# daac-tools/daachorse

Hardware: AMD Instinct MI355X
Metric: haystack GB/s scanned (find_overlapping_iter(..).count(), 100k-pattern bytewise automaton) (higher is better)
Workload: dtype u8/u32 integer

## Files before the change

### daachorse_amd/csrc/device_tables.hpp

```cpp
#pragma once

#include <hip/hip_runtime.h>

#include <cstdint>

#include "../../include/daachorse_amd.h"

namespace daac {

struct TierDev {
    const void *rows;
    const uint32_t *bcmap;
    const uint32_t *bfail;
    const uint2 *ssum;
    const uint8_t *cls;
    const uint4 *grec;
    const uint32_t *sopos;
    const uint32_t *outputs;
    const uint32_t *ohash;
    uint32_t C, NA, NB, N;
    uint32_t off_bcmap, off_bfail, off_ssum, off_cls, lds_bytes;
    uint32_t row32, root_flag;
};

struct DArrayDev {
    const uint2 *hot;
    const uint32_t *fail;
    const uint32_t *fail_plain;
    const uint4 *rec;
    const uint4 *root_chain;
    const uint4 *root;
    const uint2 *osum;
    const uint32_t *outputs;
    const uint32_t *ohash;
    uint32_t n, root_flag, leftmost;
};

struct CharDev {
    const uint4 *states;
    const uint32_t *fail_plain;
    const uint32_t *table;
    const uint2 *osum;
    const uint32_t *outputs;
    const uint32_t *ohash;
    uint32_t table_len, n, root_flag, leftmost;
    uint32_t map_in_lds;
    uint32_t map_lo;
    const uint2 *root_row;
    uint32_t alphabet;
    uint32_t row_in_lds;
    const uint4 *wstates;
    uint32_t obits, fbits;
};

struct ScanArgs {
    const uint8_t *hay;
    uint64_t begin;
    uint64_t len;
    uint64_t seg_bytes;
    uint64_t nseg;
    uint32_t halo;
    unsigned long long *result;
    unsigned long long *seg_counts;
    daac_match *out;
    uint64_t total_len;
    unsigned long long *flags;
};

struct ScanArgs;
struct ChainArgs;

struct ChainArgs {
    const unsigned long long *x_spec;
    const unsigned long long *x_prev;
    unsigned long long *x_out;
    unsigned int *flags;
    uint4 *tally_spec;
    uint4 *tally_delta;
    uint64_t cap;
};

struct GramDev {
    const uint32_t *cls32;
    const uint16_t *cid;
    const uint2 *combo;
    const uint32_t *bbits;
    const uint8_t *brank;
    const uint32_t *bsuper;
    const uint4 *drec;
    const uint2 *dhit;
    const uint4 *dhit4;
    const uint32_t *cfirst;
    uint32_t off_cid, off_combo, off_bbits, off_brank, off_bsuper, off_scratch, lds_bytes;
    uint32_t K, C, CC, CCC;
    uint32_t level_start, unused_byte, has_short;
    uint32_t rank_in_lds;
    uint32_t n_deep;
};

struct GramArgs {
    const uint8_t *hay_al;
    uint32_t lead;
    uint64_t vlen;
    uint64_t region_bytes;
    uint64_t nregions;
    unsigned long long *result;
    uint2 *wq;
    uint32_t wq_slab;
    uint32_t ppl;
    uint32_t dense;
    const uint32_t *sel;
    uint32_t sel_want;
};

hipError_t launch_gram_scan(const GramDev &dev, const GramArgs &a, uint32_t blocks, uint32_t threads, hipStream_t stream);

constexpr uint32_t kGram2OffH = 512;
struct Gram2Dev {
    const uint8_t *cls;
    const uint32_t *m;
    const void *sdir;
    const uint16_t *rfull;
    const uint16_t *cid4;
    const uint32_t *hsum;
    const uint4 *drec;
    const uint2 *dhit;
    const uint4 *dhit4;
    const uint32_t *cfirst;
    uint32_t m_bytes, s_bytes, cid_bytes, h_bytes;
    uint32_t off_m_count, off_s_count, off_ring_count, lds_count;
    uint32_t rfull_bytes, off_ring_rfull, lds_rfull, rfull_ok;
    uint32_t off_m_exact, off_s_exact, off_cid, off_ring_exact, lds_exact;
    uint32_t K, C, s16, unused_byte, n_deep, exact_ok;
    uint32_t xlane_dpp;
};
uint32_t gram2_lds_bytes(const Gram2Dev &dev, bool exact);

struct Gram2WDev {
    const uint8_t *cls;
    const unsigned long long *m;
    const uint32_t *sdir;
    const uint16_t *cid4;
    const uint32_t *hsum;
    const uint4 *drec;
    const uint4 *dhit;
    uint32_t m_bytes, s_bytes, cid_bytes, h_bytes;
    uint32_t off_m_count, off_s_count, off_ring_count, lds_count;
    uint32_t off_m_exact, off_s_exact, off_cid, off_ring_exact, lds_exact;
    uint32_t C, unused_byte, n_deep, exact_ok;
};
hipError_t launch_gram2w_scan(const Gram2WDev &dev, const GramArgs &a, bool exact, uint32_t blocks, hipStream_t stream);

constexpr uint32_t kGram2OffM = 512;
struct Gram2EmitDev {
    const uint8_t *cls;
    const uint32_t *me;
    const void *sdir;
    const uint32_t *v1, *v2;
    const uint32_t *v3;
    const uint4 *erec;
    const uint2 *ehit;
    const uint4 *ehit4;
    const uint32_t *dupo, *dupv;
    uint32_t level_start;
    const uint32_t *cfirst;
    uint32_t m_bytes, s_bytes, v1_bytes, v2_bytes;
    uint32_t off_s, off_v1, off_v2, off_ring, off_wave, lds_bytes;
    uint32_t K, C, s16, unused_byte;
    const uint32_t *v3c;
    uint32_t v3c_bytes, v3c_dir, v3c_val;
};
hipError_t launch_gram2_scan(const Gram2Dev &dev, const GramArgs &a, bool exact, uint32_t blocks, uint32_t threads, hipStream_t stream);

struct Gram3Lds {
    uint32_t off_s;
    uint32_t off_wave;
    uint32_t wave_stride;
    uint32_t lds_bytes, threads, rfull;
};

constexpr uint32_t kGram4EndsBitDev = 30;
struct Gram4Dev {
    const uint8_t *cls;
    const uint32_t *m;
    const uint16_t *rfull;
    const void *sdir;
    const uint2 *dhit_c;
    const uint4 *dhit_t;
    const uint4 *drec_c;
    const uint4 *drec_t;
    const uint32_t *bloom;
    uint32_t bloom_words;
    uint32_t m_bytes, rfull_bytes, s_bytes;
    uint32_t K, C, s16, arith, lo, unused_byte, n_deep;
};
struct Gram4Lds {
    uint32_t off_wave;
    uint32_t wave_stride;
    uint32_t off_cls;
    uint32_t off_s;
    uint32_t off_m;
    uint32_t s_bytes;
    uint32_t lds_bytes, threads;
    uint32_t arith;
    uint32_t dir;
    uint32_t filter;
    uint32_t off_b;
    uint32_t s_bytes_f;
};
uint32_t gram4_filter_room(uint32_t m_bytes, uint32_t sdir_bytes, bool arith, uint32_t lds_limit);
bool gram4_plan(const Gram4Dev &dev, uint32_t ppl, uint32_t waves, bool rfull, bool want_arith, bool want_filter, uint32_t lds_limit, Gram4Lds &L);
hipError_t launch_gram4_scan(const Gram4Dev &dev, const GramArgs &a, const Gram4Lds &L, uint32_t blocks, hipStream_t stream);

constexpr uint32_t kEmit3Tile = 1024;
constexpr uint32_t kEmit3Chunk = 1024;
constexpr uint32_t kEmit3MaxExtras = 64;
constexpr uint32_t kEmit3Stage = 960;
constexpr uint32_t kEmit3ExpandWave = (kEmit3Stage + 64) * 8 + 2048 + 256 + 1024 + kEmit3MaxExtras * 16 + 16;
constexpr uint32_t kEmit3ExpandWave16 = (kEmit3Stage + 64) * 2 + 1040 + 2048 + 256 + 1024 + kEmit3MaxExtras * 16 + 16;
struct Emit3Args {
    const uint8_t *hay_al;
    uint32_t lead;
    uint32_t vlen;
    uint32_t emit_from;
    uint8_t *ann;
    uint32_t *tile_short;
    uint32_t *tile_deep;
    uint32_t tile0;
    uint4 *recs;
    uint32_t *chunk_fill;
    uint32_t *chunk_next;
    uint32_t chunk_cap;
    uint2 *wq;
    uint32_t wq_slab;
    uint32_t region_bytes;
    uint32_t nregions;
    unsigned int *fail;
};
struct Expand3Args {
    const uint8_t *ann;
    uint32_t ntiles;
    const unsigned long long *tile_off;
    const unsigned long long *bin_off;
    const uint4 *binned;
    void *out;
    unsigned long long pos_base;
    uint32_t off_wave;
    uint32_t has_len1;
    uint32_t v3_in_lds;
    unsigned int *fail;
    uint32_t vlen, emit_from;
};
bool emit3_plan(const Gram2EmitDev &dev, uint32_t waves, uint32_t lds_limit, Gram3Lds &L);
hipError_t launch_emit3_detect(const Gram2EmitDev &dev, const Emit3Args &a, const Gram3Lds &L, uint32_t blocks, hipStream_t stream);
hipError_t launch_emit3_combine(const uint32_t *tile_short, const uint32_t *tile_deep, unsigned long long *total, unsigned long long *deep, uint64_t n,
                                hipStream_t stream);
hipError_t launch_emit3_bin(const uint4 *recs, const uint32_t *chunk_fill, const uint32_t *chunk_next, uint32_t chunk_cap, const unsigned long long *bin_off,
                            uint32_t *cursor, uint4 *binned, uint32_t n1k, unsigned long long rec_limit, uint32_t blocks, hipStream_t stream);
hipError_t launch_emit3_expand(const Gram2EmitDev &dev, const Expand3Args &a, bool f16, uint32_t blocks, hipStream_t stream);
hipError_t launch_emit3_expand_raw(const Gram2EmitDev &dev, const Expand3Args &a, bool f16, uint32_t blocks, hipStream_t stream);
uint32_t emit3_expand_lds_bytes(const Gram2EmitDev &dev, uint32_t waves, bool f16, bool v3_in_lds);

constexpr uint32_t kFind3Tile = 2048;
constexpr uint32_t kFind3Deep = 255;
constexpr uint32_t kLeft3Wave = 2080 + 4096 + 1024 + 256 + 288;
constexpr uint32_t kFind3Wave = 2064 + 4096 + 1024 + 256;
struct Find3Dev {
    const uint32_t *h1, *h2;
    const uint32_t *h3c;
    uint32_t h1_bytes, h2_bytes, h3c_bytes, h3c_dir, h3c_val, C;
};
struct Find3Args {
    const uint8_t *ann;
    uint32_t ntiles;
    uint32_t n1k;
    const unsigned long long *bin_off;
    const uint4 *binned;
    const uint32_t *entry_in;
    uint32_t *exit_out;
    uint32_t force_pos;
    unsigned long long pos_base;
    uint32_t off_wave;
    uint32_t count_only;
    unsigned long long *result;
    unsigned long long *tile_cnt;
    const unsigned long long *tile_off;
    void *out;
    uint32_t f16;
    uint32_t first_start;
    uint32_t last_start;
    uint32_t *last_sel;
    unsigned int *flag;
    const uint32_t *ctl;
    uint32_t chunk_cap;
    unsigned long long rec_limit;
};
__device__ __forceinline__ bool find3_detect_usable(const Find3Args &a) {
    return a.ctl[0] <= a.chunk_cap && a.ctl[1] == 0u && a.bin_off[a.n1k] <= a.rec_limit;
}
uint32_t find3_lds_bytes(const Find3Dev &dev, bool tally);
hipError_t launch_find3_select(const Find3Dev &dev, const Find3Args &a, bool has_len1, bool tally, uint32_t blocks, hipStream_t stream);
hipError_t launch_find3_emit(const Find3Dev &dev, const Find3Args &a, bool has_len1, uint32_t blocks, hipStream_t stream);
hipError_t launch_left3_emit(const Find3Dev &dev, const Find3Args &a, bool has_len1, uint32_t blocks, hipStream_t stream);
hipError_t launch_find3_tail(const Find3Args &a, bool has_len1, uint32_t blocks, hipStream_t stream);
uint32_t left3_lds_bytes(const Find3Dev &dev, bool tally);
hipError_t launch_left3_tail(const Find3Args &a, bool has_len1, uint32_t blocks, hipStream_t stream);
hipError_t launch_left3_select(const Find3Dev &dev, const Find3Args &a, bool has_len1, bool tally, uint32_t blocks, hipStream_t stream);

struct PfxDev {
    const uint32_t *bloom;
    const uint16_t *cnt1;
    const uint16_t *disp;
    const uint4 *slots;
    const uint2 *wrec;
    const uint4 *slots_x;
    const uint4 *wrec_x;
    const uint32_t *hs1;
    const uint4 *slots_e;
    uint32_t G, has_len1, bloom_words, buckets, n_slots, seed;
    uint32_t bloom_bytes, disp_bytes;
    uint32_t off_disp, off_cnt1, off_wave, wave_stride, lds_bytes, threads;
    uint32_t n_keys;
};
bool pfx_plan(PfxDev &d, uint32_t lds_limit);
hipError_t launch_pfx_scan(const PfxDev &dev, const GramArgs &a, bool exact, uint32_t blocks, hipStream_t stream);
hipError_t launch_pfx_probe(const PfxDev &dev, const uint8_t *hay, uint64_t len, unsigned int *out, hipStream_t stream);
struct Emit3Args;
hipError_t launch_pfx_emit_detect(const PfxDev &dev, const Emit3Args &a, uint32_t blocks, hipStream_t stream);

hipError_t launch_overlap_count(const DArrayDev &dev, const ScanArgs &a, bool heads, uint32_t blocks, hipStream_t stream);
hipError_t launch_char_overlap_count(const CharDev &dev, const ScanArgs &a, bool heads, uint32_t blocks, hipStream_t stream);
hipError_t launch_tier_scan(const TierDev &dev, const ScanArgs &a, int mode, bool heads, uint32_t blocks, uint32_t threads,
                            hipStream_t stream);
hipError_t launch_darray_scan(const DArrayDev &dev, const ScanArgs &a, int mode, bool heads, uint32_t blocks, uint32_t threads,
                              hipStream_t stream);
hipError_t launch_restart_scan(const DArrayDev &dev, const ScanArgs &a, int kmode, bool leftmost, unsigned long long *next_begin,
                               uint32_t blocks, uint32_t threads, hipStream_t stream);
hipError_t launch_char_scan(const CharDev &dev, const ScanArgs &a, int mode, bool heads, uint32_t blocks, uint32_t threads,
                            hipStream_t stream);
hipError_t launch_char_restart_scan(const CharDev &dev, const ScanArgs &a, int kmode, bool leftmost, unsigned long long *next_begin,
                                    uint32_t blocks, uint32_t threads, hipStream_t stream);
hipError_t launch_chain(const DArrayDev &dev, const ScanArgs &a, const ChainArgs &c, int pass, int kmode, bool leftmost,
                        unsigned long long *next_begin, uint32_t blocks, hipStream_t stream);
hipError_t launch_char_chain(const CharDev &dev, const ScanArgs &a, const ChainArgs &c, int pass, int kmode, bool leftmost,
                             unsigned long long *next_begin, uint32_t blocks, hipStream_t stream);
hipError_t launch_exclusive_scan(unsigned long long *v, uint64_t n, unsigned long long *total, unsigned long long *scratch, hipStream_t stream);
inline uint64_t exclusive_scan_scratch(uint64_t n) { return n / 2048 + 2; }

}
```

### daachorse_amd/csrc/gram4_kernels.hip

```cpp
#include <hip/hip_runtime.h>

#include <algorithm>
#include <cstdint>
#include <utility>

#include "device_tables.hpp"
#include "gram4_filter.hpp"

namespace daac {

namespace {

typedef uint32_t g4_u32x4_t __attribute__((ext_vector_type(4)));
constexpr uint32_t kList4 = 256;
constexpr uint32_t kProbePercent4 = 3;
typedef __attribute__((address_space(3))) const uint32_t lds4_cu32;
typedef __attribute__((address_space(3))) uint32_t lds4_u32;
typedef __attribute__((address_space(3))) const uint16_t lds4_cu16;
typedef __attribute__((address_space(3))) uint16_t lds4_u16;
typedef __attribute__((address_space(3))) const uint8_t lds4_cu8;
typedef __attribute__((address_space(3))) g4_u32x4_t lds4_u32x4;

__device__ __forceinline__ uint32_t pin4(uint32_t x) {
    asm("" : "+v"(x));
    return x;
}
__device__ __forceinline__ uint32_t mad24(uint32_t a, uint32_t b, uint32_t c) {
    uint32_t d;
    asm("v_mad_u32_u24 %0, %1, %2, %3" : "=v"(d) : "v"(a), "s"(b), "v"(c));
    return d;
}
__device__ __forceinline__ uint32_t wave_shr1_4(uint32_t v, uint32_t lane0) {
    uint32_t d = lane0;
    asm volatile("s_nop 1\nv_mov_b32_dpp %0, %1 wave_shr:1 row_mask:0xf bank_mask:0xf" : "+v"(d) : "v"(v));
    return d;
}
__device__ __forceinline__ uint32_t g4_wave_scan(uint32_t v) {
    v += static_cast<uint32_t>(__builtin_amdgcn_update_dpp(0, static_cast<int>(v), 0x111, 0xf, 0xf, false));
    v += static_cast<uint32_t>(__builtin_amdgcn_update_dpp(0, static_cast<int>(v), 0x112, 0xf, 0xf, false));
    v += static_cast<uint32_t>(__builtin_amdgcn_update_dpp(0, static_cast<int>(v), 0x114, 0xf, 0xf, false));
    v += static_cast<uint32_t>(__builtin_amdgcn_update_dpp(0, static_cast<int>(v), 0x118, 0xf, 0xf, false));
    v += static_cast<uint32_t>(__builtin_amdgcn_update_dpp(0, static_cast<int>(v), 0x142, 0xa, 0xf, false));
    v += static_cast<uint32_t>(__builtin_amdgcn_update_dpp(0, static_cast<int>(v), 0x143, 0xc, 0xf, false));
    return v;
}
template <typename F, int... I>
__device__ __forceinline__ void g4_turns(F &&f, std::integer_sequence<int, I...>) {
    (void)(... && f(std::integral_constant<int, I>{}));
}
__device__ __forceinline__ unsigned long long g4_wave_sum(unsigned long long v) {
#pragma unroll
    for (int off = 32; off > 0; off >>= 1) v += __shfl_down(v, off, 64);
    return v;
}
__device__ __forceinline__ void g4_copy(void *dst, const void *src, uint32_t bytes) {
    const uint4 *s = reinterpret_cast<const uint4 *>(src);
    uint4 *d = reinterpret_cast<uint4 *>(dst);
    for (uint32_t i = threadIdx.x; i < bytes / 16; i += blockDim.x) d[i] = s[i];
}
__device__ __forceinline__ void g4_reduce(unsigned long long cnt, unsigned long long *scratch, unsigned long long *result) {
    const unsigned long long c = g4_wave_sum(cnt);
    __syncthreads();
    const int wave = threadIdx.x >> 6, lane = threadIdx.x & 63;
    if (lane == 0) scratch[wave] = c;
    __syncthreads();
    if (threadIdx.x == 0) {
        unsigned long long r0 = 0;
        for (int w = 0; w < static_cast<int>((blockDim.x + 63) >> 6); ++w) r0 += scratch[w];
        if (r0) atomicAdd(result, r0);
    }
}

}

template <int K, int Q, bool ARITH, int DIR, bool TAIL, bool FILT>
__device__ __forceinline__ void gram4_body(const Gram4Dev &g, const GramArgs &a, const Gram4Lds &L, char *smem) {
    static_assert(!(FILT && TAIL), "the filter runs in front of the plain records");
    static_assert(!(FILT && DIR == 0), "the filter's Bloom array lies where the per-word directory would");
    constexpr int P = 16 * Q;
    constexpr int GS = 8;
    constexpr uint32_t SB = 64u * P;
    constexpr uint32_t SLOT = SB + 32u;
    const uint32_t offM = L.off_m, offS = L.off_s, offC = L.off_cls;
    const uint32_t lo = g.lo, OTH = g.C - 1u, C = g.C;
    auto cls_of = [&](uint32_t byte) -> uint32_t {
        if (ARITH) {
            const uint32_t u = byte - lo;
            return u < OTH ? u : OTH;
        }
        return *reinterpret_cast<lds4_cu8 *>(static_cast<uintptr_t>(offC + byte));
    };
    auto lds_u32 = [&](uint32_t addr) -> uint32_t { return *reinterpret_cast<lds4_cu32 *>(static_cast<uintptr_t>(addr)); };
    auto below = [&](uint32_t k) -> uint32_t { return (1u << k) - 1u; };

    const uint32_t lane = threadIdx.x & 63;
    const uint32_t wave_in_wg = __builtin_amdgcn_readfirstlane(threadIdx.x >> 6);
    const uint32_t C4 = C * 4u, CC4 = C * C * 4u;
    const uint32_t ub4 = g.unused_byte * 0x01010101u;
    const uint8_t *__restrict__ hay = a.hay_al;
    const uint64_t nwaves = static_cast<uint64_t>(gridDim.x) * (blockDim.x >> 6);
    const uint32_t tb = L.off_wave + wave_in_wg * L.wave_stride;
    const uint32_t listb = wave_in_wg * (kList4 * 2u);
    const uint64_t slab_index = (static_cast<uint64_t>(blockIdx.x) * (blockDim.x >> 6) + wave_in_wg) * a.wq_slab;
    uint4 *__restrict__ slab4 = reinterpret_cast<uint4 *>(a.wq) + slab_index;
    uint32_t wq_n = 0, slab_hi = 0;
    uint64_t epoch_base = 0;
    const uint32_t drain_early = wave_in_wg * 64u;

    unsigned long long tot_cnt = 0;
    uint32_t cnt32 = 0;

    auto load_chunk = [&](uint64_t v) -> uint4 {
        if (v >= a.vlen) return uint4{ub4, ub4, ub4, ub4};
        const g4_u32x4_t q = __builtin_nontemporal_load(reinterpret_cast<const g4_u32x4_t *>(hay + v));
        uint4 r{q.x, q.y, q.z, q.w};
        if (v < a.lead || v + 16 > a.vlen) {
            uint32_t w[4] = {r.x, r.y, r.z, r.w};
            for (int b = 0; b < 16; ++b) {
                const uint64_t p = v + b;
                if (p < a.lead || p >= a.vlen) w[b >> 2] = (w[b >> 2] & ~(0xffu << (8 * (b & 3)))) | (g.unused_byte << (8 * (b & 3)));
            }
            r = uint4{w[0], w[1], w[2], w[3]};
        }
        return r;
    };
    auto raw_at = [&](uint64_t p) -> uint32_t { return (p >= a.lead && p < a.vlen) ? hay[p] : g.unused_byte; };
    auto read_ahead = [&](uint64_t v) -> unsigned long long {
        unsigned long long x;
        if (v >= a.lead && v + 8 <= a.vlen) {
            __builtin_memcpy(&x, hay + v, 8);
        } else {
            x = 0;
            for (int b = 7; b >= 0; --b) x = (x << 8) | ((v + b >= a.lead && v + b < a.vlen) ? hay[v + b] : g.unused_byte);
        }
        return x;
    };
    auto tail_count = [&](const uint4 &rr, unsigned long long text) -> uint32_t {
        const uint32_t edges = rr.x & 15u;
        const unsigned long long path = (static_cast<unsigned long long>(rr.w) << 32) | rr.z;
        const unsigned long long diff = path ^ text;
        uint32_t same = diff ? static_cast<uint32_t>(__builtin_ctzll(diff)) >> 3 : 8u;
        same = same < edges ? same : edges;
        return __popc((rr.x >> 4) & ((2u << same) - 1u) & 0x1ffu);
    };
    auto drain = [&]() {
        const uint4 *__restrict__ recs = TAIL ? g.drec_t : g.drec_c;
        uint32_t n_in = wq_n;
        bool raw = !TAIL;
        while (n_in != 0) {
            uint32_t n_out = 0;
            for (uint32_t base = 0; base < n_in; base += 64u) {
                const uint32_t i = base + lane;
                const bool live = i < n_in;
                uint4 e = uint4{0u, 0u, 0u, 0u};
                if (live) e = slab4[i];
                uint32_t state, n_ahead;
                unsigned long long ah;
                if (raw) {
                    const uint32_t k1 = cls_of(e.w & 0xffu);
                    state = e.z + __popc(e.y & below(k1));
                    ah = e.w >> 8;
                    n_ahead = 3;
                } else {
                    state = e.y & 0x07ffffffu;
                    ah = (static_cast<unsigned long long>(e.w & 0xffffffu) << 32) | e.z;
                    n_ahead = e.w >> 24;
                }
                uint4 rr = uint4{0u, 0u, 0u, 0u};
                if (live) rr = recs[state];
                const uint64_t vn = epoch_base + e.x + 2;
                bool cont = false;
                uint32_t next_state = 0;
                if (rr.x >> 31) {
                    if (n_ahead < (rr.x & 15u)) ah = read_ahead(vn);
                    cnt32 += tail_count(rr, ah);
                } else {
                    if (live && n_ahead == 0u) { ah = read_ahead(vn); n_ahead = 8; }
                    const uint32_t k = cls_of(static_cast<uint32_t>(ah) & 0xffu);
                    cnt32 += rr.z;
                    cont = ((rr.x >> k) & 1u) != 0;
                    next_state = rr.y + __popc(rr.x & below(k));
                }
                const unsigned long long m = __ballot(cont);
                if (m != 0) {
                    if (cont) {
                        const uint32_t at = n_out + __builtin_amdgcn_mbcnt_hi(static_cast<uint32_t>(m >> 32), __builtin_amdgcn_mbcnt_lo(static_cast<uint32_t>(m), 0));
                        ah >>= 8;
                        slab4[at] = uint4{e.x + 1u, next_state, static_cast<uint32_t>(ah), static_cast<uint32_t>(ah >> 32) | ((n_ahead - 1u) << 24)};
                    }
                    n_out += static_cast<uint32_t>(__popcll(m));
                }
            }
            n_in = n_out;
            raw = false;
        }
        wq_n = 0;
    };

    uint32_t q_head = 0, q_tail = 0;
    uint32_t posbias = 0;
    uint32_t st_n = 0;
    uint32_t pend_lo = 0;
    uint4 pend = uint4{0u, 0u, 0u, 0u};
    uint32_t pend_pos = 0;
    uint32_t pend_t0 = 0, pend_t1 = 0;
    bool pend_valid = false;
    uint4 p2 = uint4{0u, 0u, 0u, 0u};
    uint32_t p2_pos = 0, p2_state = 0;
    uint32_t p2_t0 = 0, p2_t1 = 0;
    bool p2_live = false, p2_any = false;
    uint32_t sb_n = 0;
    uint32_t sb_pos = 0, sb_lo = 0, sb_t0 = 0;
    uint32_t fp_pos = 0, fp_t0 = 0;
    const uint32_t offB = L.off_b, bloomW = g.bloom_words;
    auto push_walker = [&](bool go, const uint4 &entry) {
        const unsigned long long m = __ballot(go);
        if (m != 0) {
            if (go) {
                const uint32_t at = wq_n + __builtin_amdgcn_mbcnt_hi(static_cast<uint32_t>(m >> 32), __builtin_amdgcn_mbcnt_lo(static_cast<uint32_t>(m), 0));
                slab4[at] = entry;
            }
            wq_n += __popcll(m);
        }
    };
    auto finish_second = [&]() {
        if (!TAIL || !p2_any) return;
        p2_any = false;
        const uint4 r = p2;
        bool again = false;
        uint32_t st_k = 0, pos = p2_pos, t0 = p2_t0, t1n = (p2_t1 & 0xffffffu) | (7u << 24);
        if (p2_live) {
            if (r.x >> 31) {
                if ((r.x & 15u) <= 7u) cnt32 += tail_count(r, (static_cast<unsigned long long>(p2_t1) << 32) | p2_t0);
                else { again = true; st_k = p2_state; }
            } else {
                cnt32 += r.z;
                const uint32_t k = p2_state >> 27;
                if ((r.x >> k) & 1u) {
                    again = true;
                    const uint32_t k3 = cls_of((p2_t0 >> 8) & 0xffu);
                    st_k = (r.y + __popc(r.x & below(k))) | (k3 << 27);
                    pos = p2_pos + 1u;
                    t0 = __builtin_amdgcn_alignbyte(p2_t1, p2_t0, 1u);
                    t1n = ((p2_t1 >> 8) & 0xffffu) | (6u << 24);
                }
            }
        }
        p2_live = false;
        push_walker(again, uint4{pos, st_k, t0, t1n});
    };
    auto consume_pending = [&]() {
        finish_second();
        if (!pend_valid) return;
        pend_valid = false;
        const uint4 r = pend;
        if (FILT) {
            const uint32_t k1 = cls_of(fp_t0 & 0xffu);
            cnt32 += (r.x >> kGram4EndsBitDev) & 1u;
            push_walker(__builtin_amdgcn_ubfe(r.x, k1, 1) != 0, uint4{fp_pos, r.x, r.y, fp_t0});
            return;
        }
        const uint32_t k1 = cls_of(pend_t0 & 0xffu);
        if (!TAIL) {
            cnt32 += (r.x >> kGram4EndsBitDev) & 1u;
            push_walker(__builtin_amdgcn_ubfe(r.x, k1, 1) != 0, uint4{pend_pos, r.x, r.y, pend_t0});
            return;
        }
        bool go;
        if (r.x >> 31) {
            cnt32 += tail_count(r, (static_cast<unsigned long long>(pend_t1) << 32) | pend_t0);
            go = false;
        } else {
            cnt32 += (r.x >> kGram4EndsBitDev) & 1u;
            go = ((r.x >> k1) & 1u) != 0;
        }
        p2 = uint4{0u, 0u, 0u, 0u};
        p2_live = go;
        p2_any = __ballot(go) != 0;
        if (go) {
            const uint32_t child = r.y + __popc(r.x & below(k1));
            const uint32_t k2 = cls_of((pend_t0 >> 8) & 0xffu);
            p2 = g.drec_t[child];
            p2_pos = pend_pos;
            p2_state = child | (k2 << 27);
            p2_t0 = __builtin_amdgcn_alignbyte(pend_t1, pend_t0, 1u);
            p2_t1 = pend_t1 >> 8;
        }
    };
    auto derive = [&](uint32_t first, uint32_t cnt) {
        if (lane - first < cnt) {
            const uint32_t e = tb + *reinterpret_cast<lds4_cu16 *>(static_cast<uintptr_t>(listb + ((q_head + lane - first) << 1)));
            pend_pos = e + posbias;
            const uint32_t t3 = e - 3u;
            const uint32_t a0 = t3 & ~3u, sh = t3 & 3u;
            const uint32_t d0 = lds_u32(a0), d1 = lds_u32(a0 + 4u), d2 = lds_u32(a0 + 8u);
            pend_lo = __builtin_amdgcn_alignbyte(d1, d0, sh);
            pend_t0 = __builtin_amdgcn_alignbyte(d2, d1, sh);
            if (TAIL) {
                const uint32_t d3 = lds_u32(a0 + 12u);
                pend_t1 = __builtin_amdgcn_alignbyte(d3, d2, sh);
            }
        }
        q_head += cnt;
    };
    const uint32_t lo_idx = K == 3 ? lo * (C * C + C + 1u) : lo * (C + 1u);
    auto rank_and_ask = [&](uint32_t x_lo) {
        uint32_t idx, d;
        if (ARITH) {
            idx = mad24((x_lo >> 8) & 0xffu, C, ((x_lo >> 16) & 0xffu) - lo_idx);
            if (K == 3) idx = mad24(x_lo & 0xffu, C * C, idx);
            d = (x_lo >> 24) - lo;
        } else {
            const uint32_t c1 = cls_of((x_lo >> 8) & 0xffu), c2 = cls_of((x_lo >> 16) & 0xffu);
            d = cls_of(x_lo >> 24);
            idx = __umul24(c1, C) + c2;
            if (K == 3) idx = __umul24(cls_of(x_lo & 0xffu), C * C) + idx;
        }
        const uint32_t am = (idx << 2) + offM;
        const uint32_t own = lds_u32(am);
        uint32_t rank;
        if (DIR == 0) {
            const uint32_t base = *reinterpret_cast<lds4_cu16 *>(static_cast<uintptr_t>((idx << 1) + offS));
            rank = base + __popc(own & below(d));
        } else {
            const uint32_t grp = am & ~15u;
            const uint32_t qx = lds_u32(grp), qy = lds_u32(grp + 4u), qz = lds_u32(grp + 8u);
            const uint32_t gi = pin4(idx >> 2);
            const uint32_t base = DIR == 1 ? *reinterpret_cast<lds4_cu16 *>(static_cast<uintptr_t>((gi << 1) + offS))
                                           : *reinterpret_cast<lds4_cu32 *>(static_cast<uintptr_t>((gi << 2) + offS));
            const uint32_t mx = static_cast<uint32_t>(__builtin_amdgcn_sbfe(static_cast<int>(0xEEEEEEEEu), idx, 1u));
            const uint32_t my = static_cast<uint32_t>(__builtin_amdgcn_sbfe(static_cast<int>(0xCCCCCCCCu), idx, 1u));
            const uint32_t mz = static_cast<uint32_t>(__builtin_amdgcn_sbfe(static_cast<int>(0x88888888u), idx, 1u));
            uint32_t under = __popc(own & below(d));
            under += __popc(qx & mx & 0x3fffffffu);
            under += __popc(qy & my & 0x3fffffffu);
            under += __popc(qz & mz & 0x3fffffffu);
            rank = base + under;
        }
        if (TAIL) {
            pend = g.dhit_t[rank];
        } else {
            const uint2 h = g.dhit_c[rank];
            pend = uint4{h.x, h.y, 0u, 0u};
        }
    };
    auto survivors_ask = [&](uint32_t n) {
        consume_pending();
        pend = uint4{0u, 0u, 0u, 0u};
        if (lane < n) rank_and_ask(sb_lo);
        fp_pos = sb_pos;
        fp_t0 = lane < n ? sb_t0 : 0u;
        pend_valid = true;
    };
    auto process_batch = [&](uint32_t n) {
        __builtin_amdgcn_s_setprio(2);
        if (FILT) {
            derive(st_n, n - st_n);
            st_n = 0;
            const G4Probe pr = g4f_probe(K == 3 ? pend_lo : pend_lo >> 8, pend_t0 & 0xffu, bloomW);
            const uint32_t fw = lds_u32(offB + (pr.word << 2));
            const bool pass = lane < n && ((pr.go & ~fw) == 0u || (pr.ends & ~fw) == 0u);
            const unsigned long long pm = __builtin_amdgcn_ballot_w64(pass);
            if (pm != 0) {
                const uint32_t s = static_cast<uint32_t>(__popcll(pm));
                const uint32_t r = __builtin_amdgcn_mbcnt_hi(static_cast<uint32_t>(pm >> 32), __builtin_amdgcn_mbcnt_lo(static_cast<uint32_t>(pm), 0));
                uint32_t t;
                asm("v_cndmask_b32_e64 %0, 63, %1, %2" : "=v"(t) : "v"(r), "s"(pm));
                const uint32_t tgt = ((t + sb_n) << 2) & 0xfcu;
                const uint32_t r_pos = static_cast<uint32_t>(__builtin_amdgcn_ds_permute(static_cast<int>(tgt), static_cast<int>(pend_pos)));
                const uint32_t r_lo = static_cast<uint32_t>(__builtin_amdgcn_ds_permute(static_cast<int>(tgt), static_cast<int>(pend_lo)));
                const uint32_t r_t0 = static_cast<uint32_t>(__builtin_amdgcn_ds_permute(static_cast<int>(tgt), static_cast<int>(pend_t0)));
                const bool mine = lane - sb_n < s;
                sb_pos = mine ? r_pos : sb_pos;
                sb_lo = mine ? r_lo : sb_lo;
                sb_t0 = mine ? r_t0 : sb_t0;
                if (sb_n + s >= 64u) {
                    survivors_ask(64u);
                    sb_pos = r_pos; sb_lo = r_lo; sb_t0 = r_t0;
                    sb_n = sb_n + s - 64u;
                } else {
                    sb_n += s;
                }
            }
            return;
        }
        consume_pending();
        derive(st_n, n - st_n);
        st_n = 0;
        pend = uint4{0u, 0u, 0u, 0u};
        if (lane < n) {
            rank_and_ask(pend_lo);
        } else {
            pend_t0 = 0;
            pend_t1 = 0;
        }
        pend_valid = true;
    };

    uint64_t region = static_cast<uint64_t>(blockIdx.x) * (blockDim.x >> 6) + wave_in_wg;
    while (region < a.nregions) {
      slab_hi = static_cast<uint32_t>((region * a.region_bytes) >> 31);
      epoch_base = static_cast<uint64_t>(slab_hi) << 31;
      for (; region < a.nregions && static_cast<uint32_t>((region * a.region_bytes) >> 31) == slab_hi; region += nwaves) {
        const uint64_t rbase = region * a.region_bytes;
        const uint64_t rend = rbase + a.region_bytes < a.vlen ? rbase + a.region_bytes : a.vlen;
        uint32_t carry = 0, tail4 = 0;
#pragma unroll
        for (int i = 0; i < K; ++i) carry |= (rbase >= static_cast<uint64_t>(K - i) ? cls_of(raw_at(rbase - (K - i))) : OTH) << (8 * i);
#pragma unroll
        for (int i = 0; i < 4; ++i) tail4 |= (rbase >= static_cast<uint64_t>(4 - i) ? raw_at(rbase - (4 - i)) : static_cast<uint32_t>(g.unused_byte)) << (8 * i);
        tail4 = __builtin_amdgcn_readfirstlane(tail4);
        carry = __builtin_amdgcn_readfirstlane(carry);
        uint32_t mcarry;
        {
            uint32_t x = (((carry >> (8 * (K - 1))) & 0xffu) << 2) + offM;
            x += __umul24((carry >> (8 * (K - 2))) & 0xffu, C4);
            if (K == 3) x += __umul24(carry & 0xffu, CC4);
            mcarry = __builtin_amdgcn_readfirstlane(lds_u32(x));
        }

        auto fetch = [&](uint64_t s0, uint4 (&out)[Q]) {
#pragma unroll
            for (int q = 0; q < Q; ++q) out[q] = uint4{ub4, ub4, ub4, ub4};
            if (s0 < rend) {
#pragma unroll
                for (int q = 0; q < Q; ++q) out[q] = load_chunk(s0 + lane * P + 16u * q);
            } else if (lane == 0 && s0 < rend + SB) {
                out[0] = load_chunk(s0);
            }
        };
        uint4 pf0[Q], pf1[Q];
        fetch(rbase, pf0);
        fetch(rbase + SB, pf1);

        for (uint64_t sb = rbase; sb < rend; sb += SB) {
            if (wq_n + 64u * P + 128u + drain_early > a.wq_slab) drain();
            uint4 cur[Q];
#pragma unroll
            for (int q = 0; q < Q; ++q) { cur[q] = pf0[q]; pf0[q] = pf1[q]; }
            consume_pending();
            __builtin_amdgcn_s_setprio(0);
            fetch(sb + 2ull * SB, pf1);

            if (q_tail != q_head) {
                const uint32_t n_left = q_tail - q_head;
                derive(st_n, n_left);
                st_n += n_left;
            }
            q_head = q_tail = 0;
            const uint32_t slot = tb;
            const uint32_t my_text = slot + 16u + lane * P;
            posbias = static_cast<uint32_t>(sb - epoch_base) - (slot + 16u);
#pragma unroll
            for (int q = 0; q < Q; ++q)
                *reinterpret_cast<lds4_u32x4 *>(static_cast<uintptr_t>(my_text + 16u * q)) = g4_u32x4_t{cur[q].x, cur[q].y, cur[q].z, cur[q].w};
            if (lane == 0) {
                *reinterpret_cast<lds4_u32 *>(static_cast<uintptr_t>(slot + 12u)) = tail4;
                *reinterpret_cast<lds4_u32x4 *>(static_cast<uintptr_t>(slot + 16u + SB)) = g4_u32x4_t{pf0[0].x, pf0[0].y, pf0[0].z, pf0[0].w};
            }
            tail4 = __builtin_amdgcn_readlane(cur[Q - 1].w, 63);

            uint32_t kx[K + P];
#pragma unroll
            for (int q = 0; q < Q; ++q) {
                const uint32_t w[4] = {cur[q].x, cur[q].y, cur[q].z, cur[q].w};
#pragma unroll
                for (int b = 0; b < 16; ++b) {
                    kx[K + 16 * q + b] = pin4(cls_of((w[b >> 2] >> (8 * (b & 3))) & 0xffu));
                    __builtin_assume(kx[K + 16 * q + b] < 32u);
                }
            }
            uint32_t pk = 0;
#pragma unroll
            for (int i = 0; i < K; ++i) pk |= kx[P + i] << (8 * i);
            const uint32_t left = wave_shr1_4(pk, carry);
            carry = __builtin_amdgcn_readlane(pk, 63);
#pragma unroll
            for (int i = 0; i < K; ++i) { kx[i] = (left >> (8 * i)) & 0xffu; __builtin_assume(kx[i] < 32u); }

            uint32_t H = 0, ccnt = 0, roll = 0, mprev = 0;
#pragma unroll
            for (int grp = 0; grp < P / GS; ++grp) {
                uint32_t mw[GS];
#pragma unroll
                for (int jj = 0; jj < GS; ++jj) {
                    const int j = grp * GS + jj;
                    uint32_t x = pin4((kx[K + j] << 2) + offM);
                    x = mad24(kx[K + j - 1], C4, x);
                    if (K == 3) x = mad24(kx[K + j - 2], CC4, x);
                    mw[jj] = lds_u32(x);
                }
#pragma unroll
                for (int jj = 0; jj < GS; ++jj) {
                    const int j = grp * GS + jj;
                    roll = __builtin_amdgcn_alignbit(roll, mw[jj], 30);
                    if (j > 0) H = __builtin_amdgcn_alignbit((jj == 0 ? mprev : mw[jj - 1]) >> kx[K + j], H, 1);
                    if ((j & 15) == 15) {
                        ccnt += __popc(roll & 0x55555555u) + 2u * __popc(roll & 0xaaaaaaaau);
                        roll = 0;
                    }
                }
                mprev = mw[GS - 1];
            }
            {
                const uint32_t mleft = wave_shr1_4(mprev, mcarry);
                mcarry = __builtin_amdgcn_readlane(mprev, 63);
                H |= __builtin_amdgcn_ubfe(mleft, kx[K], 1) << (32 - P);
            }
            cnt32 += ccnt;

            const uint32_t text_adj = my_text - (32u - P) - tb;
            for (;;) {
                if (__ballot(H != 0u) == 0) break;
                const uint32_t n = __popc(H);
                const uint32_t incl = g4_wave_scan(n);
                const uint32_t tot = __builtin_amdgcn_readlane(incl, 63);
                const uint32_t first = q_tail + incl - n;
                const uint32_t room = first < kList4 ? kList4 - first : 0u;
                const uint32_t lim = n < room ? n : room;
                const uint32_t at = pin4(listb + (first << 1));
                g4_turns([&](auto tc) -> bool {
                    constexpr uint32_t t = decltype(tc)::value;
                    const bool w = t < lim;
                    if (__ballot(w) == 0) return false;
                    if (w) {
                        *reinterpret_cast<lds4_u16 *>(static_cast<uintptr_t>(at + 2u * t)) = static_cast<uint16_t>(text_adj + __builtin_ctz(H));
                        H &= H - 1u;
                    }
                    return true;
                }, std::make_integer_sequence<int, P>{});
                const uint32_t in = std::min(tot, kList4 - q_tail);
                q_tail += in;
                while (st_n + q_tail - q_head >= 64u) process_batch(64u);
                if (in == tot) break;
                const uint32_t n_left = q_tail - q_head;
                if (lane < n_left) {
                    const uint16_t v = *reinterpret_cast<lds4_cu16 *>(static_cast<uintptr_t>(listb + ((q_head + lane) << 1)));
                    *reinterpret_cast<lds4_u16 *>(static_cast<uintptr_t>(listb + (lane << 1))) = v;
                }
                q_head = 0;
                q_tail = n_left;
            }
        }
        tot_cnt += cnt32;
        cnt32 = 0;
      }
      if (st_n + q_tail - q_head != 0) process_batch(st_n + q_tail - q_head);
      if (FILT && sb_n != 0) { survivors_ask(sb_n); sb_n = 0; }
      consume_pending();
      finish_second();
      drain();
      tot_cnt += cnt32;
      cnt32 = 0;
    }
    g4_reduce(tot_cnt, reinterpret_cast<unsigned long long *>(smem), a.result);
}

template <int K, int Q, bool ARITH, int DIR, int TPB, bool FILT>
__global__ __launch_bounds__(TPB) void gram4_kernel(const Gram4Dev g, const GramArgs a, const Gram4Lds L) {
    extern __shared__ __attribute__((aligned(16))) char smem[];
    constexpr int DIRC = DIR == 0 ? 1 : DIR;
    if (!ARITH) g4_copy(smem + L.off_cls, g.cls, 256);
    g4_copy(smem + L.off_m, g.m, g.m_bytes);
    uint32_t *votes = reinterpret_cast<uint32_t *>(smem + L.off_wave);
    if (threadIdx.x == 0) *votes = 0;
    __syncthreads();
    if (__builtin_amdgcn_groupstaticsize() != 0) __builtin_trap();
    bool tail = a.sel_want == 1u;
    if (a.sel_want == 2u) {
        const uint64_t span = a.vlen > a.lead + 16 ? a.vlen - a.lead - 8 : 0;
        bool go = false;
        if (span != 0) {
            unsigned long long h = (static_cast<unsigned long long>(threadIdx.x) + 1) * 0x9E3779B97F4A7C15ull;
            h ^= h >> 29;
            const uint64_t p = a.lead + 3 + (h % (span - 3));
            const uint8_t *t = a.hay_al + p;
            const uint32_t OTH = g.C - 1u;
            auto cl = [&](uint32_t b) -> uint32_t {
                if (ARITH) { const uint32_t u = b - g.lo; return u < OTH ? u : OTH; }
                return reinterpret_cast<const uint8_t *>(smem + L.off_cls)[b];
            };
            const uint32_t *m = reinterpret_cast<const uint32_t *>(smem + L.off_m);
            const uint32_t c0 = cl(t[-3]), c1 = cl(t[-2]), c2 = cl(t[-1]), d = cl(t[0]), k1 = cl(t[1]);
            const uint32_t ctx = K == 3 ? (c0 * g.C + c1) * g.C + c2 : c1 * g.C + c2;
            const uint32_t w = m[ctx];
            if ((w >> d) & 1u & (d < OTH ? 1u : 0u)) {
                uint32_t rank = __popc(w & ((1u << d) - 1u));
                for (uint32_t j = ctx & ~3u; j < ctx; ++j) rank += __popc(m[j] & 0x3fffffffu);
                rank += g.s16 ? reinterpret_cast<const uint16_t *>(g.sdir)[ctx >> 2] : reinterpret_cast<const uint32_t *>(g.sdir)[ctx >> 2];
                const uint2 r = g.dhit_c[rank];
                go = ((r.x >> k1) & 1u) != 0;
            }
        }
        const unsigned long long bm = __ballot(go);
        if ((threadIdx.x & 63) == 0 && bm != 0) atomicAdd(votes, static_cast<uint32_t>(__popcll(bm)));
        __syncthreads();
        tail = *votes * 100u > static_cast<uint32_t>(TPB) * kProbePercent4;
        __syncthreads();
    }
    if (FILT && !tail) {
        g4_copy(smem + L.off_s, g.sdir, L.s_bytes_f);
        g4_copy(smem + L.off_b, g.bloom, g.bloom_words * 4u);
    } else {
        g4_copy(smem + L.off_s, DIR == 0 ? static_cast<const void *>(g.rfull) : g.sdir, L.s_bytes);
    }
    __syncthreads();
    if (tail) gram4_body<K, Q, ARITH, DIR, true, false>(g, a, L, smem);
    else if constexpr (FILT) gram4_body<K, Q, ARITH, DIRC, false, true>(g, a, L, smem);
    else gram4_body<K, Q, ARITH, DIR, false, false>(g, a, L, smem);
}

template <int K, int Q, bool ARITH, int DIR, int TPB, bool FILT>
static hipError_t launch4_inst(const Gram4Dev &dev, const GramArgs &a, const Gram4Lds &L, uint32_t blocks, hipStream_t stream) {
    const hipError_t e = hipFuncSetAttribute(reinterpret_cast<const void *>(gram4_kernel<K, Q, ARITH, DIR, TPB, FILT>),
                                             hipFuncAttributeMaxDynamicSharedMemorySize, static_cast<int>(L.lds_bytes));
    if (e != hipSuccess) return e;
    hipLaunchKernelGGL((gram4_kernel<K, Q, ARITH, DIR, TPB, FILT>), dim3(blocks), dim3(TPB), L.lds_bytes, stream, dev, a, L);
    return hipGetLastError();
}
template <int K, int Q, int TPB, bool ARITH>
static hipError_t launch4_d(const Gram4Dev &dev, const GramArgs &a, const Gram4Lds &L, uint32_t blocks, hipStream_t stream) {
    if (L.filter) {
        if (L.dir == 0) return launch4_inst<K, Q, ARITH, 0, TPB, true>(dev, a, L, blocks, stream);
        if (L.dir == 1) return launch4_inst<K, Q, ARITH, 1, TPB, true>(dev, a, L, blocks, stream);
        return launch4_inst<K, Q, ARITH, 2, TPB, true>(dev, a, L, blocks, stream);
    }
    if (L.dir == 0) return launch4_inst<K, Q, ARITH, 0, TPB, false>(dev, a, L, blocks, stream);
    if (L.dir == 1) return launch4_inst<K, Q, ARITH, 1, TPB, false>(dev, a, L, blocks, stream);
    return launch4_inst<K, Q, ARITH, 2, TPB, false>(dev, a, L, blocks, stream);
}
template <int K, int Q, int TPB>
static hipError_t launch4_k(const Gram4Dev &dev, const GramArgs &a, const Gram4Lds &L, uint32_t blocks, hipStream_t stream) {
    return L.arith ? launch4_d<K, Q, TPB, true>(dev, a, L, blocks, stream) : launch4_d<K, Q, TPB, false>(dev, a, L, blocks, stream);
}

bool gram4_plan(const Gram4Dev &dev, uint32_t ppl, uint32_t waves, bool rfull, bool want_arith, bool want_filter, uint32_t lds_limit, Gram4Lds &L) {
    L = Gram4Lds{};
    if (rfull && dev.rfull == nullptr) return false;
    const uint32_t slot = 64u * ppl + 32u;
    L.wave_stride = slot;
    L.off_wave = waves * kList4 * 2u;
    L.threads = waves * 64u;
    L.arith = (want_arith && dev.arith) ? 1u : 0u;
    const uint32_t per_wg = L.off_wave + waves * L.wave_stride;
    L.off_cls = per_wg;
    L.off_s = per_wg + (L.arith ? 0u : 256u);
    L.dir = rfull ? 0u : (dev.s16 ? 1u : 2u);
    L.s_bytes = rfull ? dev.rfull_bytes : dev.s_bytes;
    uint32_t region = L.s_bytes;
    if (want_filter && dev.bloom != nullptr) {
        const uint32_t with = dev.s_bytes + dev.bloom_words * 4u;
        if (L.off_s + std::max(region, with) + dev.m_bytes <= lds_limit) {
            L.filter = 1u;
            L.s_bytes_f = dev.s_bytes;
            L.off_b = L.off_s + dev.s_bytes;
            region = std::max(region, with);
        }
    }
    L.off_m = L.off_s + region;
    L.lds_bytes = L.off_m + dev.m_bytes;
    return L.lds_bytes <= lds_limit;
}
uint32_t gram4_filter_room(uint32_t m_bytes, uint32_t sdir_bytes, bool arith, uint32_t lds_limit) {
    const uint32_t fixed = 16u * kList4 * 2u + 16u * (64u * 32u + 32u) + (arith ? 0u : 256u) + sdir_bytes + m_bytes;
    return fixed < lds_limit ? (lds_limit - fixed) & ~15u : 0u;
}

hipError_t launch_gram4_scan(const Gram4Dev &dev, const GramArgs &a, const Gram4Lds &L, uint32_t blocks, hipStream_t stream) {
    if (a.ppl == 32 && L.threads == 1024)
        return dev.K == 3 ? launch4_k<3, 2, 1024>(dev, a, L, blocks, stream) : launch4_k<2, 2, 1024>(dev, a, L, blocks, stream);
    if (a.ppl == 32)
        return dev.K == 3 ? launch4_k<3, 2, 512>(dev, a, L, blocks, stream) : launch4_k<2, 2, 512>(dev, a, L, blocks, stream);
    if (L.threads == 512)
        return dev.K == 3 ? launch4_k<3, 1, 512>(dev, a, L, blocks, stream) : launch4_k<2, 1, 512>(dev, a, L, blocks, stream);
    return dev.K == 3 ? launch4_k<3, 1, 1024>(dev, a, L, blocks, stream) : launch4_k<2, 1, 1024>(dev, a, L, blocks, stream);
}

}
```

Measured before the change: 1629.

## Compute packed gram indices with u16 SIMD ops and place mask table at LDS zero

New measurement: 1652, median of 6. 1.4% higher.

```diff
diff --git a/daachorse_amd/csrc/device_tables.hpp b/daachorse_amd/csrc/device_tables.hpp
--- a/daachorse_amd/csrc/device_tables.hpp
+++ b/daachorse_amd/csrc/device_tables.hpp
@@ -200,6 +200,7 @@
     uint32_t off_cls;
     uint32_t off_s;
     uint32_t off_m;
+    uint32_t off_list;
     uint32_t s_bytes;
     uint32_t lds_bytes, threads;
     uint32_t arith;
diff --git a/daachorse_amd/csrc/gram4_kernels.hip b/daachorse_amd/csrc/gram4_kernels.hip
--- a/daachorse_amd/csrc/gram4_kernels.hip
+++ b/daachorse_amd/csrc/gram4_kernels.hip
@@ -28,6 +28,41 @@
 __device__ __forceinline__ uint32_t mad24(uint32_t a, uint32_t b, uint32_t c) {
     uint32_t d;
     asm("v_mad_u32_u24 %0, %1, %2, %3" : "=v"(d) : "v"(a), "s"(b), "v"(c));
+    return d;
+}
+__device__ __forceinline__ uint32_t pk_sub_u16(uint32_t a, uint32_t s) {
+    uint32_t d;
+    asm("v_pk_sub_u16 %0, %1, %2" : "=v"(d) : "v"(a), "s"(s));
+    return d;
+}
+__device__ __forceinline__ uint32_t pk_min_u16(uint32_t a, uint32_t s) {
+    uint32_t d;
+    asm("v_pk_min_u16 %0, %1, %2" : "=v"(d) : "v"(a), "s"(s));
+    return d;
+}
+__device__ __forceinline__ uint32_t pk_mad_u16(uint32_t a, uint32_t s, uint32_t c) {
+    uint32_t d;
+    asm("v_pk_mad_u16 %0, %1, %2, %3" : "=v"(d) : "v"(a), "s"(s), "v"(c));
+    return d;
+}
+__device__ __forceinline__ uint32_t lo16x4(uint32_t x) {
+    uint32_t d;
+    asm("v_lshlrev_b32_sdwa %0, 2, %1 dst_sel:DWORD dst_unused:UNUSED_PAD src0_sel:DWORD src1_sel:WORD_0" : "=v"(d) : "v"(x));
+    return d;
+}
+__device__ __forceinline__ uint32_t hi16x4(uint32_t x) {
+    uint32_t d;
+    asm("v_lshlrev_b32_sdwa %0, 2, %1 dst_sel:DWORD dst_unused:UNUSED_PAD src0_sel:DWORD src1_sel:WORD_1" : "=v"(d) : "v"(x));
+    return d;
+}
+__device__ __forceinline__ uint32_t shr_lo16(uint32_t m, uint32_t s) {
+    uint32_t d;
+    asm("v_lshrrev_b32 %0, %1, %2" : "=v"(d) : "v"(s), "v"(m));
+    return d;
+}
+__device__ __forceinline__ uint32_t shr_hi16(uint32_t m, uint32_t s) {
+    uint32_t d;
+    asm("v_lshrrev_b32_sdwa %0, %1, %2 dst_sel:DWORD dst_unused:UNUSED_PAD src0_sel:WORD_1 src1_sel:DWORD" : "=v"(d) : "v"(s), "v"(m));
     return d;
 }
 __device__ __forceinline__ uint32_t wave_shr1_4(uint32_t v, uint32_t lane0) {
@@ -81,7 +116,8 @@
     constexpr int GS = 8;
     constexpr uint32_t SB = 64u * P;
     constexpr uint32_t SLOT = SB + 32u;
-    const uint32_t offM = L.off_m, offS = L.off_s, offC = L.off_cls;
+    constexpr uint32_t offM = 0;
+    const uint32_t offS = L.off_s, offC = L.off_cls;
     const uint32_t lo = g.lo, OTH = g.C - 1u, C = g.C;
     auto cls_of = [&](uint32_t byte) -> uint32_t {
         if (ARITH) {
@@ -96,11 +132,12 @@
     const uint32_t lane = threadIdx.x & 63;
     const uint32_t wave_in_wg = __builtin_amdgcn_readfirstlane(threadIdx.x >> 6);
     const uint32_t C4 = C * 4u, CC4 = C * C * 4u;
+    const uint32_t lo2 = lo * 0x10001u, oth2 = OTH * 0x10001u, c2 = C * 0x10001u;
     const uint32_t ub4 = g.unused_byte * 0x01010101u;
     const uint8_t *__restrict__ hay = a.hay_al;
     const uint64_t nwaves = static_cast<uint64_t>(gridDim.x) * (blockDim.x >> 6);
     const uint32_t tb = L.off_wave + wave_in_wg * L.wave_stride;
-    const uint32_t listb = wave_in_wg * (kList4 * 2u);
+    const uint32_t listb = L.off_list + wave_in_wg * (kList4 * 2u);
     const uint64_t slab_index = (static_cast<uint64_t>(blockIdx.x) * (blockDim.x >> 6) + wave_in_wg) * a.wq_slab;
     uint4 *__restrict__ slab4 = reinterpret_cast<uint4 *>(a.wq) + slab_index;
     uint32_t wq_n = 0, slab_hi = 0;
@@ -418,6 +455,10 @@
             if (K == 3) x += __umul24(carry & 0xffu, CC4);
             mcarry = __builtin_amdgcn_readfirstlane(lds_u32(x));
         }
+        if (ARITH) {
+            const uint32_t k1 = (carry >> (8 * (K - 1))) & 0xffu, k2 = (carry >> (8 * (K - 2))) & 0xffu;
+            carry = K == 3 ? k1 | ((k2 * C + k1) << 16) : k1 << 16;
+        }
 
         auto fetch = [&](uint64_t s0, uint4 (&out)[Q]) {
 #pragma unroll
@@ -460,41 +501,87 @@
             }
             tail4 = __builtin_amdgcn_readlane(cur[Q - 1].w, 63);
 
-            uint32_t kx[K + P];
-#pragma unroll
-            for (int q = 0; q < Q; ++q) {
-                const uint32_t w[4] = {cur[q].x, cur[q].y, cur[q].z, cur[q].w};
-#pragma unroll
-                for (int b = 0; b < 16; ++b) {
-                    kx[K + 16 * q + b] = pin4(cls_of((w[b >> 2] >> (8 * (b & 3))) & 0xffu));
-                    __builtin_assume(kx[K + 16 * q + b] < 32u);
-                }
-            }
-            uint32_t pk = 0;
-#pragma unroll
-            for (int i = 0; i < K; ++i) pk |= kx[P + i] << (8 * i);
-            const uint32_t left = wave_shr1_4(pk, carry);
-            carry = __builtin_amdgcn_readlane(pk, 63);
-#pragma unroll
-            for (int i = 0; i < K; ++i) { kx[i] = (left >> (8 * i)) & 0xffu; __builtin_assume(kx[i] < 32u); }
-
-            uint32_t H = 0, ccnt = 0, roll = 0, mprev = 0;
-#pragma unroll
-            for (int grp = 0; grp < P / GS; ++grp) {
-                uint32_t mw[GS];
-#pragma unroll
-                for (int jj = 0; jj < GS; ++jj) {
-                    const int j = grp * GS + jj;
+            uint32_t kx[ARITH ? 1 : K + P];
+            uint32_t ce[ARITH ? P / 4 : 1], co[ARITH ? P / 4 : 1];
+            uint32_t ie[ARITH ? P / 4 : 1], io[ARITH ? P / 4 : 1];
+            if constexpr (ARITH) {
+                uint32_t w[P / 4];
+#pragma unroll
+                for (int q = 0; q < Q; ++q) { w[4 * q] = cur[q].x; w[4 * q + 1] = cur[q].y; w[4 * q + 2] = cur[q].z; w[4 * q + 3] = cur[q].w; }
+#pragma unroll
+                for (int d = 0; d < P / 4; ++d) {
+                    ce[d] = pk_min_u16(pk_sub_u16(w[d] & 0x00ff00ffu, lo2), oth2);
+                    co[d] = pk_min_u16(pk_sub_u16(__builtin_amdgcn_perm(w[d], w[d], 0x0c030c01u), lo2), oth2);
+                }
+                uint32_t t13[P / 4];
+#pragma unroll
+                for (int d = 0; d < P / 4; ++d) t13[d] = pk_mad_u16(ce[d], c2, co[d]);
+                const uint32_t mine = K == 3 ? __builtin_amdgcn_perm(t13[P / 4 - 1], co[P / 4 - 1], 0x07060302u) : co[P / 4 - 1];
+                const uint32_t left = wave_shr1_4(mine, carry);
+                carry = __builtin_amdgcn_readlane(mine, 63);
+#pragma unroll
+                for (int d = 0; d < P / 4; ++d) {
+                    const uint32_t xc = d > 0 ? __builtin_amdgcn_alignbyte(co[d], co[d - 1], 2u)
+                                              : K == 3 ? __builtin_amdgcn_perm(co[0], left, 0x05040100u) : __builtin_amdgcn_alignbyte(co[0], left, 2u);
+                    const uint32_t t02 = pk_mad_u16(xc, c2, ce[d]);
+                    if (K == 3) {
+                        const uint32_t xt = __builtin_amdgcn_alignbyte(t13[d], d > 0 ? t13[d - 1] : left, 2u);
+                        ie[d] = pk_mad_u16(xt, c2, ce[d]);
+                        io[d] = pk_mad_u16(t02, c2, co[d]);
+                    } else {
+                        ie[d] = t02;
+                        io[d] = t13[d];
+                    }
+                }
+            } else {
+#pragma unroll
+                for (int q = 0; q < Q; ++q) {
+                    const uint32_t w[4] = {cur[q].x, cur[q].y, cur[q].z, cur[q].w};
+#pragma unroll
+                    for (int b = 0; b < 16; ++b) {
+                        kx[K + 16 * q + b] = pin4(cls_of((w[b >> 2] >> (8 * (b & 3))) & 0xffu));
+                        __builtin_assume(kx[K + 16 * q + b] < 32u);
+                    }
+                }
+                uint32_t pk = 0;
+#pragma unroll
+                for (int i = 0; i < K; ++i) pk |= kx[P + i] << (8 * i);
+                const uint32_t left = wave_shr1_4(pk, carry);
+                carry = __builtin_amdgcn_readlane(pk, 63);
+#pragma unroll
+                for (int i = 0; i < K; ++i) { kx[i] = (left >> (8 * i)) & 0xffu; __builtin_assume(kx[i] < 32u); }
+            }
+            auto m_addr = [&](int j) -> uint32_t {
+                if constexpr (ARITH) {
+                    const uint32_t v = (j & 1) ? io[j >> 2] : ie[j >> 2];
+                    return (j & 2) ? hi16x4(v) : lo16x4(v);
+                } else {
                     uint32_t x = pin4((kx[K + j] << 2) + offM);
                     x = mad24(kx[K + j - 1], C4, x);
                     if (K == 3) x = mad24(kx[K + j - 2], CC4, x);
-                    mw[jj] = lds_u32(x);
-                }
+                    return x;
+                }
+            };
+            auto shr_cls = [&](uint32_t m, int j) -> uint32_t {
+                if constexpr (ARITH) {
+                    const uint32_t v = (j & 1) ? co[j >> 2] : ce[j >> 2];
+                    return (j & 2) ? shr_hi16(m, v) : shr_lo16(m, v);
+                } else {
+                    return m >> kx[K + j];
+                }
+            };
+
+            uint32_t H = 0, ccnt = 0, roll = 0, mprev = 0;
+#pragma unroll
+            for (int grp = 0; grp < P / GS; ++grp) {
+                uint32_t mw[GS];
+#pragma unroll
+                for (int jj = 0; jj < GS; ++jj) mw[jj] = lds_u32(m_addr(grp * GS + jj));
 #pragma unroll
                 for (int jj = 0; jj < GS; ++jj) {
                     const int j = grp * GS + jj;
                     roll = __builtin_amdgcn_alignbit(roll, mw[jj], 30);
-                    if (j > 0) H = __builtin_amdgcn_alignbit((jj == 0 ? mprev : mw[jj - 1]) >> kx[K + j], H, 1);
+                    if (j > 0) H = __builtin_amdgcn_alignbit(shr_cls(jj == 0 ? mprev : mw[jj - 1], j), H, 1);
                     if ((j & 15) == 15) {
                         ccnt += __popc(roll & 0x55555555u) + 2u * __popc(roll & 0xaaaaaaaau);
                         roll = 0;
@@ -505,7 +592,7 @@
             {
                 const uint32_t mleft = wave_shr1_4(mprev, mcarry);
                 mcarry = __builtin_amdgcn_readlane(mprev, 63);
-                H |= __builtin_amdgcn_ubfe(mleft, kx[K], 1) << (32 - P);
+                H |= __builtin_amdgcn_ubfe(mleft, ARITH ? ce[0] : kx[K], 1) << (32 - P);
             }
             cnt32 += ccnt;
 
@@ -639,7 +726,9 @@
     if (rfull && dev.rfull == nullptr) return false;
     const uint32_t slot = 64u * ppl + 32u;
     L.wave_stride = slot;
-    L.off_wave = waves * kList4 * 2u;
+    L.off_m = 0;
+    L.off_list = (dev.m_bytes + 15u) & ~15u;
+    L.off_wave = L.off_list + waves * kList4 * 2u;
     L.threads = waves * 64u;
     L.arith = (want_arith && dev.arith) ? 1u : 0u;
     const uint32_t per_wg = L.off_wave + waves * L.wave_stride;
@@ -650,15 +739,14 @@
     uint32_t region = L.s_bytes;
     if (want_filter && dev.bloom != nullptr) {
         const uint32_t with = dev.s_bytes + dev.bloom_words * 4u;
-        if (L.off_s + std::max(region, with) + dev.m_bytes <= lds_limit) {
+        if (L.off_s + std::max(region, with) <= lds_limit) {
             L.filter = 1u;
             L.s_bytes_f = dev.s_bytes;
             L.off_b = L.off_s + dev.s_bytes;
             region = std::max(region, with);
         }
     }
-    L.off_m = L.off_s + region;
-    L.lds_bytes = L.off_m + dev.m_bytes;
+    L.lds_bytes = L.off_s + region;
     return L.lds_bytes <= lds_limit;
 }
 uint32_t gram4_filter_room(uint32_t m_bytes, uint32_t sdir_bytes, bool arith, uint32_t lds_limit) {
```
